# vklyukin/nf_distillation

Measured on NVIDIA B200. Metric: kd_train_samples_per_sec, higher is better.
Workload: dtype bf16

## Files before the change

include/nfk.h:

```cpp
#ifndef NFK_H_
#define NFK_H_

#ifdef __cplusplus
extern "C" {
#endif

#define NFK_OK 0
#define NFK_ERR_SHAPE (-1)
#define NFK_ERR_ALIGN (-2)
#define NFK_ERR_ARG (-3)
#define NFK_ERR_LAUNCH (-4)
#define NFK_ERR_DRIVER (-5)

#define NFK_EPI_F32 0
#define NFK_EPI_BIAS_RELU_BF16 1
#define NFK_EPI_MASK_BF16 2

int nfk_version(void);

int nfk_gemm_nt_bf16(const void* A, long long lda, const void* B, long long ldb, int M, int N, int K, int epi,
                     void* out, long long ldo, const float* bias, const void* aux, long long ldaux, float* colsum,
                     void* stream);

int nfk_gemm_set_prof(void* buf);
// ... 86 lines not shown
                            const float* g_z1_sq, const float* g_ld, float* dx, float* dw, float* dbias, float* dlogs,
                            int B, int C, int H, int W, void* stream);
int nfk_dequant_squeeze(const void* src, int src_is_u8, int n_bits, const float* noise, float* x_out, float* sq_out,
                        int B, int C, int H, int W, void* stream);
int nfk_prior_bpd_fwd(const float* z, const float* mean, const float* logs, const float* logdet, int B, int n,
                      float scale, float* out, void* stream);
int nfk_prior_bpd_bwd(const float* z, const float* mean, const float* logs, const float* g_bpd, int B, int n,
                      float scale, float* dz, float* dlogdet, void* stream);
int nfk_kd_mse_fwd(const float* s, const float* t, int B, int n, float scale, float* acc, void* stream);
int nfk_kd_mse_bwd(const float* s, const float* t, const float* g, int B, int n, float scale, float* ds,
                   int accumulate, void* stream);

int nfk_pconv_coupling_supported(int C, int H, int W, int hid);
int nfk_pconv_coupling_fwd(const void* h2, const void* B3, int K3p, const float* bias3, float* y, float* hsave,
                           float* ld, int B, int C, int H, int W, int hid, int reverse, void* stream);

int nfk_conv1_dgrad_affine_bwd_supported(int C, int H, int W, int hid);
int nfk_conv1_dgrad_affine_bwd(const void* dpre1, const void* B1T, int K1p, const float* dy, const float* x,
                               const float* Wf, float* dx, float* dWf, float* dbf, int B, int C, int H, int W, int hid,
                               void* stream);

int nfk_flow1d_supported(int D, int Cc, int hid, int training);
int nfk_flow1d_sizes(int D, int Cc, int hid, int* total_fwd, int* total_bwd, int* total_grad, int* n_act,
                     int* offsets);
int nfk_flow1d_pack(const float* Wf, const float* bf, const float* const* w, const float* const* b, int D, int Cc,
                    int hid, float* PF, float* PB, void* stream);
int nfk_flow1d_fwd(const float* x, const float* cond, const float* PF, const float* sl, float* y, const float* ld_in,
                   float* ld_out, float* acts, int B, int D, int Cc, int hid, int reverse, void* stream);
int nfk_flow1d_bwd(const float* x_in, const float* cond, const float* acts, const float* PB, const float* y_out,
                   const float* g_out, const float* g_ld, float* dx, float* G, int B, int D, int Cc, int hid,
// ... 80 lines not shown
```

nf_distillation_b200/_lib.py:

```python
from __future__ import annotations

import ctypes
import os

from . import build as _build

_c = ctypes
_vp, _i, _ll, _f = _c.c_void_p, _c.c_int, _c.c_longlong, _c.c_float

ERRORS = {
    -1: "NFK_ERR_SHAPE (unsupported / inconsistent sizes)",
    -2: "NFK_ERR_ALIGN (pointer or leading dimension not 16-byte aligned)",
    -3: "NFK_ERR_ARG (missing / invalid argument)",
    -4: "NFK_ERR_LAUNCH (CUDA launch failure)",
    -5: "NFK_ERR_DRIVER (tensor-map encode failure)",
}



class InvconvItem(_c.Structure):
    _fields_ = [(n, _vp) for n in ("an_bias", "an_logs", "lower", "upper", "log_s", "p", "sign_s", "weight")] + \
               [("C", _i), ("reverse", _i), ("transpose", _i)] + \
               [(n, _vp) for n in ("outW", "outb", "out_sl")]

# ... 54 lines not shown
    "nfk_kd_mse_fwd": [_vp, _vp, _i, _i, _f, _vp, _vp],
    "nfk_kd_mse_bwd": [_vp, _vp, _vp, _i, _i, _f, _vp, _i, _vp],
    "nfk_flow1d_supported": [_i, _i, _i, _i],
    "nfk_flow1d_sizes": [_i, _i, _i, _vp, _vp, _vp, _vp, _vp],
    "nfk_flow1d_pack": [_vp, _vp, _vp, _vp, _i, _i, _i, _vp, _vp, _vp],
    "nfk_flow1d_fwd": [_vp] * 8 + [_i] * 5 + [_vp],
    "nfk_flow1d_bwd": [_vp] * 9 + [_i] * 5 + [_vp],
    "nfk_affine_rows": [_vp] * 7 + [_i, _i, _f, _vp],
    "nfk_gemm_nt_bf16_ranged": [_vp, _ll, _vp, _ll, _i, _i, _i, _i, _vp, _ll, _vp, _vp, _ll, _vp, _i, _vp, _vp, _vp],
    "nfk_cnet_set_prof": [_vp],
    "nfk_cnet_fwd_fused": [_vp, _i, _vp, _vp, _vp, _vp, _vp, _vp, _vp, _vp, _ll, _i, _i, _vp],
    "nfk_cnet_bwd_fused": [_vp, _i, _vp, _vp, _vp, _vp, _ll, _vp, _vp, _vp, _vp, _i, _i, _vp],
    "nfk_cnet_fwd_fused_ranged": [_vp, _i, _vp, _vp, _vp, _vp, _vp, _vp, _vp, _vp, _ll, _i, _i, _i, _vp],
    "nfk_pconv_coupling_supported": [_i, _i, _i, _i],
    "nfk_pconv_coupling_fwd": [_vp, _vp, _i, _vp, _vp, _vp, _vp, _i, _i, _i, _i, _i, _i, _vp],
    "nfk_conv1_dgrad_affine_bwd_supported": [_i, _i, _i, _i],
    "nfk_conv1_dgrad_affine_bwd": [_vp] * 9 + [_i] * 5 + [_vp],
    "nfk_made_prep": [_vp] * 5 + [_i] * 4 + [_vp] * 6 + [_i, _vp],
    "nfk_made_prep_bwd": [_vp] * 5 + [_i] * 3 + [_vp] * 3 + [_vp],
    "nfk_rows_to_bf16": [_vp, _i, _i, _i, _vp, _vp],
    "nfk_made_affine_fwd": [_vp, _vp, _i, _vp, _vp, _i, _vp, _vp, _i, _i, _i, _vp],
    "nfk_made_affine_bwd": [_vp, _vp, _i, _vp, _vp, _vp, _vp, _vp, _i, _i, _i, _vp],
    "nfk_made_inv_update": [_vp, _vp, _i, _vp, _vp, _i, _vp, _vp, _i, _i, _i, _i, _i, _vp],
    "nfk_made_inverse_resident_supported": [_i, _i, _i],
    "nfk_made_inverse_push_supported": [_i, _i, _i, _i],
    "nfk_made_inverse_jobs": [_vp, _vp, _i, _i, _i, _i, _i, _vp, _i],
    "nfk_made_inverse_pack": [_vp, _i, _vp, _vp, _vp, _i, _i, _i, _i, _i, _vp, _vp],
    "nfk_made_inverse_resident": [_vp] * 6 + [_i] * 3 + [_vp] * 3 + [_i] * 6 + [_vp],
    "nfk_kd_nll_loss_scratch_floats": [_i],
    "nfk_kd_nll_loss_fwd": [_vp, _vp, _i, _vp, _vp, _vp, _f, _vp, _vp, _vp, _f, _f, _f, _i, _vp, _vp, _vp, _vp, _vp],
# ... 49 lines not shown
```

nf_distillation_b200/csrc/pconv_coupling.cu:

```cuda
#include <cuda.h>
#include <cuda_bf16.h>
#include <cuda_runtime.h>
#include <cstdint>
#include <cstdlib>

#include "../../include/nfk.h"
#include "launch_util.h"
#include "ptx.cuh"

namespace nfk {

constexpr int PC_EPI = 384;
constexpr int PC_THREADS = 64 + PC_EPI;
constexpr int PC_BK = 64;

template <int C> struct PcCfg;
template <> struct PcCfg<12> { static constexpr int NPIX = 256, MB = 1, WIN = 160, STAGES = 3; };
template <> struct PcCfg<24> { static constexpr int NPIX = 128, MB = 2, WIN = 64, STAGES = 3; };
template <> struct PcCfg<48> { static constexpr int NPIX = 64, MB = 4, WIN = 32, STAGES = 2; };

struct PcArgs {
  long long M;
  int num_kb;
  int B, H, W, lgHW, lgW;
  const float* bias3;
  float* y;
  float* hsave;
  float* ld;
  int reverse;
  int banded, nb, rb;
};

template <int NPIX>
__device__ __forceinline__ long long pc_tile_pix0(const PcArgs& g, int t) {
  if (!g.banded) return static_cast<long long>(t) * NPIX;
  const int img = t / g.nb, band = t - img * g.nb;
  return (static_cast<long long>(img) << g.lgHW) + static_cast<long long>(band * g.rb - 1) * g.W;
}

template <int C>
struct PcSmem {
  using Cfg = PcCfg<C>;
  static constexpr int a_bytes = Cfg::MB * 128 * 128;
  static constexpr int b_bytes = Cfg::NPIX * 128;
  static constexpr int stage_bytes = a_bytes + b_bytes;
  static constexpr int pitch = Cfg::WIN + 1;
  static constexpr int s_bytes = ((9 * C * pitch * 4 + 15) / 16) * 16;
  static constexpr int off_s = Cfg::STAGES * stage_bytes;
  static constexpr int off_bar = off_s + s_bytes;
  static constexpr int off_bias = off_bar + 128;
  static constexpr int total = off_bias + 128;
};

template <int C>
__global__ void __launch_bounds__(PC_THREADS, 1)
pconv_coupling_kernel(const __grid_constant__ CUtensorMap tmW, const __grid_constant__ CUtensorMap tmH,
                      const PcArgs g) {
  using Cfg = PcCfg<C>;
  using Sm = PcSmem<C>;
  constexpr int NPIX = Cfg::NPIX, MB = Cfg::MB, WIN = Cfg::WIN, HALF = NPIX / 2, PC_STAGES = Cfg::STAGES;
  constexpr int K3 = 9 * C, J = C / 2;
  constexpr int ACC_COLS = MB * NPIX;
  extern __shared__ __align__(1024) uint8_t smem[];
  pdl_launch_dependents();
  if (smem_u32(smem) & 1023u) __trap();
  const int warp = static_cast<int>(uniform_u32(threadIdx.x >> 5)), lane = threadIdx.x & 31;
  float* S = reinterpret_cast<float*>(smem + Sm::off_s);
  uint64_t* full = reinterpret_cast<uint64_t*>(smem + Sm::off_bar);
  uint64_t* empty = full + PC_STAGES;
// ... 1 lines not shown
  uint64_t* tmem_empty = tmem_full + 2;
  uint32_t* tmem_slot = reinterpret_cast<uint32_t*>(tmem_empty + 2);
  float* bias_s = reinterpret_cast<float*>(smem + Sm::off_bias);

  const int num_tiles = g.banded ? g.B * g.nb : static_cast<int>((g.M + NPIX - 1) / NPIX);
  if (warp == 0 && lane == 0) {
    tma_prefetch_desc(&tmW);
    tma_prefetch_desc(&tmH);
    for (int s = 0; s < PC_STAGES; ++s) { mbar_init(&full[s], 1); mbar_init(&empty[s], 1); }
    for (int a = 0; a < 2; ++a) { mbar_init(&tmem_full[a], 1); mbar_init(&tmem_empty[a], 8); }
    fence_mbar_init();
  }
  if (warp == 1) { tmem_alloc(tmem_slot, 512); tmem_relinquish(); }
  pdl_wait();
  if (threadIdx.x < C) bias_s[threadIdx.x] = g.bias3[threadIdx.x];
  tc_fence_before();
  __syncthreads();
  tc_fence_after();
  const uint32_t tmem_base = uniform_u32(*tmem_slot);

  if (warp == 0) {
    {
      int s = 0;
      uint32_t ph = 0;
      for (int t = blockIdx.x; t < num_tiles; t += gridDim.x) {
        for (int kb = 0; kb < g.num_kb; ++kb) {
          mbar_wait_warp(&empty[s], ph ^ 1);
          uint8_t* sa = smem + s * Sm::stage_bytes;
          mbar_expect_tx_elect(&full[s], Sm::stage_bytes);
#pragma unroll
// ... 30 lines not shown
          umma_commit_elect(&empty[s]);
          if (++s == PC_STAGES) { s = 0; ph ^= 1; }
        }
        umma_commit_elect(&tmem_full[acc]);
      }
    }
  } else {
    const int q = warp & 3, half = (warp - 2) >> 2;
    const int et = threadIdx.x - 64;
    const bool drains = half < 2;
    const bool banded = (C == 12) && g.banded;
    const int HW = g.H * g.W, HWm = HW - 1, Wm = g.W - 1;
    constexpr int ITEMS = J * NPIX / PC_EPI;
    static_assert(J * NPIX % (2 * PC_EPI) == 0, "each half's items must divide over the epilogue threads");
    const int OH = banded ? (g.rb >> 1) * g.W : HALF;
    int it = 0;
    for (int t = blockIdx.x; t < num_tiles; t += gridDim.x, ++it) {
      const int acc = it & 1;
      const long long tile_base = pc_tile_pix0<NPIX>(g, t);
      const int row0 = banded ? (t % g.nb) * g.rb - 1 : 0;
      const int row_end = banded ? min(g.H, row0 + 1 + g.rb) : 0;
      auto decode = [&](int hf, int ih, int& j, int& pl, long long& m) -> bool {
        j = ih / OH;
        pl = (banded ? g.W : 0) + hf * OH + (ih - j * OH);
        m = tile_base + pl;
        if (j >= J) return false;
        if (!banded) return m < g.M;
        return row0 + (pl >> g.lgW) < row_end;
      };
      float z2v[ITEMS];
#pragma unroll
      for (int k = 0; k < ITEMS; ++k) {
        const int hf = k / (ITEMS / 2);
        int j, pl;
        long long m;
        const bool live = decode(hf, et + PC_EPI * (k - hf * (ITEMS / 2)), j, pl, m);
        const int b = static_cast<int>(m >> g.lgHW), rem = static_cast<int>(m) & HWm;
        z2v[k] = live ? g.y[((static_cast<long long>(b) * C + J + j) << g.lgHW) + rem] : 0.f;
      }
      mbar_wait(&tmem_full[acc], (it >> 1) & 1);
      tc_fence_after();
#pragma unroll
      for (int hf = 0; hf < 2; ++hf) {
        const int w0 = (WIN == HALF) ? hf * HALF : (hf == 0 ? 0 : NPIX - WIN);
        if (hf == 1) asm volatile("bar.sync 1, %0;" ::"n"(PC_EPI) : "memory");
        constexpr int HCOLS = WIN / 2;
        static_assert(HCOLS % 16 == 0, "window halves are drained 16 columns at a time");
#pragma unroll
        for (int mb = 0; mb < MB; ++mb) {
          const int row = mb * 128 + q * 32 + lane;
          const uint32_t taddr = tmem_base + (static_cast<uint32_t>(q * 32) << 16) + acc * ACC_COLS + mb * NPIX + w0 +
                                 half * HCOLS;
          float* srow = S + row * Sm::pitch + half * HCOLS;
// ... 40 lines not shown
              const int dy = tap / 3 - 1, dx = tap % 3 - 1;
              const int ny = yy + dy, nx = xx + dx;
              if (ny >= 0 && ny < g.H && nx >= 0 && nx < g.W) {
                const float* p = sp + tap * C * Sm::pitch + dy * g.W + dx;
                sh += p[0];
                lg += p[Sm::pitch];
              }
            }
            if (g.hsave) *reinterpret_cast<float2*>(g.hsave + m * C + 2 * j) = make_float2(sh, lg);
            const float tt = lg + 2.f;
            const float e = expf(-fabsf(tt));
            const float l1p = log1pf(e);
            float sg, lsv;
            if (tt >= 0.f) { sg = 1.f / (1.f + e); lsv = -l1p; }
            else { sg = e / (1.f + e); lsv = tt - l1p; }
            g.y[((static_cast<long long>(b) * C + J + j) << g.lgHW) + rem] =
                g.reverse ? (z2v[k] / sg - sh) : (z2v[k] + sh) * sg;
            lsum = g.reverse ? -lsv : lsv;
          }
          if (g.ld) {
            const int seg = HW < 32 ? HW : 32;
#pragma unroll
            for (int o = 16; o > 0; o >>= 1) {
              const float v = __shfl_xor_sync(0xffffffffu, lsum, o);
              if (o < seg) lsum += v;
            }
            if ((lane & (seg - 1)) == 0 && live) atomicAdd(g.ld + b, lsum);
          }
        }
      }
      asm volatile("bar.sync 1, %0;" ::"n"(PC_EPI) : "memory");
    }
  }
  tc_fence_before();
  __syncthreads();
  if (warp == 1) tmem_dealloc(tmem_base, 512);
}

typedef CUresult (*EncodeTiledFn3)(CUtensorMap*, CUtensorMapDataType, cuuint32_t, void*, const cuuint64_t*,
                                   const cuuint64_t*, const cuuint32_t*, const cuuint32_t*, CUtensorMapInterleave,
                                   CUtensorMapSwizzle, CUtensorMapL2promotion, CUtensorMapFloatOOBfill);

int pc_tmap(CUtensorMap* m, const void* ptr, uint64_t cols, uint64_t rows, uint64_t ld, uint32_t box_rows) {
// ... 5 lines not shown
        q != cudaDriverEntryPointSuccess)
      return NFK_ERR_DRIVER;
    fn = reinterpret_cast<EncodeTiledFn3>(p);
  }
  if ((reinterpret_cast<uintptr_t>(ptr) & 15) || (ld * 2) % 16) return NFK_ERR_ALIGN;
  cuuint64_t dims[2] = {cols, rows};
  cuuint64_t strides[1] = {ld * 2};
  cuuint32_t box[2] = {64, box_rows};
  cuuint32_t estr[2] = {1, 1};
  CUresult r = fn(m, CU_TENSOR_MAP_DATA_TYPE_BFLOAT16, 2, const_cast<void*>(ptr), dims, strides, box, estr,
                  CU_TENSOR_MAP_INTERLEAVE_NONE, CU_TENSOR_MAP_SWIZZLE_128B, CU_TENSOR_MAP_L2_PROMOTION_L2_256B,
                  CU_TENSOR_MAP_FLOAT_OOB_FILL_NONE);
  return r == CUDA_SUCCESS ? NFK_OK : NFK_ERR_DRIVER;
}

template <int C>
static int pc_launch(const void* h2, const void* B3, int K3p, const PcArgs& g, int hid, cudaStream_t st) {
  using Cfg = PcCfg<C>;
  CUtensorMap tmW, tmH;
  int rc;
  if ((rc = pc_tmap(&tmW, B3, hid, K3p, hid, 128))) return rc;
  if ((rc = pc_tmap(&tmH, h2, hid, static_cast<uint64_t>(g.M), hid, Cfg::NPIX))) return rc;
  if ((rc = ensure_dyn_smem(reinterpret_cast<const void*>(pconv_coupling_kernel<C>), PcSmem<C>::total))) return rc;
  int dev = 0, sms = 148;
  cudaGetDevice(&dev);
  cudaDeviceGetAttribute(&sms, cudaDevAttrMultiProcessorCount, dev);
  const int tiles = g.banded ? g.B * g.nb : static_cast<int>((g.M + Cfg::NPIX - 1) / Cfg::NPIX);
  const cudaError_t le = launch_pdl(pconv_coupling_kernel<C>, dim3(tiles < sms ? tiles : sms), dim3(PC_THREADS),
                                    PcSmem<C>::total, st, tmW, tmH, g);
  return (le == cudaSuccess && cudaGetLastError() == cudaSuccess) ? NFK_OK : NFK_ERR_LAUNCH;
}

int pconv_px_launch(const void* h2, const void* B3, int K3p, const float* bias3, float* y, float* hsave, float* ld,
                    int B, int C, int hid, int reverse, cudaStream_t st);
static bool pconv_use_px() {
  static const bool v = [] { const char* e = getenv("NFK_PCONV_PX"); return !(e && e[0] == '0'); }();
  return v;
}

}

using namespace nfk;

extern "C" int nfk_pconv_coupling_supported(int C, int H, int W, int hid) {
  if (hid <= 0 || hid % 64) return 0;
  const int HW = H * W;
  if (HW < 4 || (HW & (HW - 1)) || (W & (W - 1))) return 0;
  if (C == 12) {
    if (HW <= PcCfg<12>::NPIX / 2) return 1;
    if (HW == PcCfg<12>::NPIX && W + 1 <= PcCfg<12>::WIN - PcCfg<12>::NPIX / 2) return 1;
    return W * 8 == PcCfg<12>::NPIX && 3 * W + W + 1 <= PcCfg<12>::WIN + 1;
  }
  if (C == 24) return HW <= PcCfg<24>::NPIX / 2 && HW >= 4;
  if (C == 48) return HW <= PcCfg<48>::NPIX / 2 && HW >= 4;
  if (C == 96) return H == 4 && W == 4 && pconv_use_px();
  return 0;
}

extern "C" int nfk_pconv_coupling_fwd(const void* h2, const void* B3, int K3p, const float* bias3, float* y,
                                      float* hsave, float* ld, int B, int C, int H, int W, int hid, int reverse,
                                      void* stream) {
  if (B <= 0 || !nfk_pconv_coupling_supported(C, H, W, hid)) return NFK_ERR_SHAPE;
  if (K3p % 64 || K3p < 9 * C || K3p > 128 * ((9 * C + 127) / 128)) return NFK_ERR_SHAPE;
  if (!h2 || !B3 || !bias3 || !y) return NFK_ERR_ARG;
  PcArgs g{};
  g.M = static_cast<long long>(B) * H * W;
  g.num_kb = hid / 64;
  g.B = B; g.H = H; g.W = W;
  g.lgW = 0; while ((1 << g.lgW) < W) ++g.lgW;
  g.lgHW = 0; while ((1 << g.lgHW) < H * W) ++g.lgHW;
  g.bias3 = bias3; g.y = y; g.hsave = hsave; g.ld = ld; g.reverse = reverse;
// ... 13 lines not shown
```

nf_distillation_b200/functional.py:

```python
from __future__ import annotations

import os
from dataclasses import dataclass
from typing import Optional

import torch

from . import ops

BF16 = torch.bfloat16
F32 = torch.float32
USE_FUSED_CNET = os.environ.get("NFK_FUSED_CNET", "1") != "0"
USE_FUSED_PCONV = os.environ.get("NFK_FUSED_PCONV", "1") != "0"
USE_FUSED_CNET_BWD = os.environ.get("NFK_FUSED_CNET_BWD", "1") != "0"
USE_FUSED_DGRAD1 = os.environ.get("NFK_FUSED_DGRAD1", "1") != "0"

WGRAD_STREAM_MAX_M = int(os.environ.get("NFK_WGRAD_STREAM_MAX_M", "65536"))
_wgrad_streams: dict = {}
_wgrad_keepalive: list = []


def _wgrad_stream(dev):
    key = (dev.type, dev.index if dev.index is not None else torch.cuda.current_device())
    st = _wgrad_streams.get(key)
    if st is None:
        st = _wgrad_streams[key] = torch.cuda.Stream(device=dev)
    return st


def _join_wgrads(dev):
# ... 41 lines not shown


class PrepCtx:

    def __init__(self, steps, reverse: bool):
        self.steps = list(steps)
        self.reverse = bool(reverse)
        self.index = {id(s): i for i, s in enumerate(self.steps)}
        n = len(self.steps)
        self.consts = [None] * n
        self.items = [None] * n
        self.grads = [None] * n
        self.cops = [None] * n
        self.citems = [None] * n
        self.cgrads = [None] * n
        self.token = None

    def build(self):
        flat = []
        for st in self.steps:
            iv = st.invconv
            if iv.LU_decomposed:
                flat += [st.actnorm.bias, st.actnorm.logs, iv.lower, iv.upper, iv.log_s]
            else:
                flat += [st.actnorm.bias, st.actnorm.logs, iv.weight, iv.weight, iv.weight]
        for st in self.steps:
            if not st.is_1d:
                flat += list(st._coupling_params_2d())
        self.token = PrepAllFn.apply(self, *flat)
        return self
# ... 174 lines not shown
        ops.gemm_nt(col, k.B1, M, hid, K1p, ops.EPI_BIAS_RELU_BF16, h1, bias=k.bias1, aux=m1)
        ops.gemm_nt(h1, k.B2, M, hid, hid, ops.EPI_BIAS_RELU_BF16, h2, bias=k.bias2, aux=m2)
    return (h1, h2, m1, m2) if keep else (None, h2, None, None)


def _conv3_coupling(h2, k: StepConsts, y, hsave, ld, B, C, H, W, hid, K3p, reverse):
    M = B * H * W
    if USE_FUSED_PCONV and ops.pconv_coupling_supported(C, H, W, hid):
        ops.pconv_coupling_fwd(h2, k.B3, K3p, k.bias3, y, hsave, ld, B, C, H, W, hid, reverse)
        return
    P = torch.empty(M, K3p, device=h2.device, dtype=F32)
    ops.gemm_nt(h2, k.B3, M, K3p, hid, ops.EPI_F32, P)
    ops.coupling_fwd(P, K3p, k.bias3, y, hsave, ld, B, C, H, W, reverse=reverse)


def flowstep2d_forward(x, ld_in, k: StepConsts, hid, keep):
    B, C, H, W = x.shape
    M, cin = B * H * W, C // 2
    K1p, K3p = ops.round_up(9 * cin, 64), ops.round_up(9 * C, 64)
    dev = x.device
    y = torch.empty_like(x)
    col = torch.empty(M, K1p, device=dev, dtype=BF16)
    ld_out = torch.empty(B, device=dev, dtype=F32)
    ops.affine1x1_fwd(x, k.Wf, k.bf, k.sl, y, col, K1p, ld_in, ld_out, B, C, H, W)
    h1, h2, m1, m2 = _coupling_net(col, k, M, hid, K1p, K3p, keep)
    hsave = torch.empty(M, C, device=dev, dtype=F32) if keep else None
    _conv3_coupling(h2, k, y, hsave, ld_out, B, C, H, W, hid, K3p, False)
    return y, ld_out, (col, h1, h2 if keep else None, hsave, m1, m2)


def flowstep2d_reverse(z, ld_in, k: StepConsts, hid, keep=False):
    B, C, H, W = z.shape
    M, cin = B * H * W, C // 2
    K1p, K3p = ops.round_up(9 * cin, 64), ops.round_up(9 * C, 64)
    dev = z.device
    col = torch.empty(M, K1p, device=dev, dtype=BF16)
    ops.affine1x1_fwd(z, None, None, None, None, col, K1p, None, None, B, C, H, W)
    h1, h2, m1, m2 = _coupling_net(col, k, M, hid, K1p, K3p, keep)
    hsave = torch.empty(M, C, device=dev, dtype=F32) if keep else None
    zc = z.clone()
    ld_mid = ld_in.clone()
    _conv3_coupling(h2, k, zc, hsave, ld_mid, B, C, H, W, hid, K3p, True)
# ... 38 lines not shown
        ops.gemm_tn(dhcol, h2, K3p, hid, M, dB3)
        ops.gemm_tn(dpre2, h1, hid, hid, M, dB2)
        ops.gemm_tn(dpre1, col, hid, K1p, M, dB1)
    return dpre1


def _conv1_dgrad(dpre1, B1T, M, K1p, hid):
    dcol = torch.empty(M, K1p, device=dpre1.device, dtype=F32)
    ops.gemm_nt(dpre1, B1T, M, K1p, hid, ops.EPI_F32, dcol)
    return dcol


class FlowStep2dFn(torch.autograd.Function):

    @staticmethod
    def forward(ctx, x, ld_in, hid, token, pctx, idx):
        B, C, H, W = x.shape
        x = x.contiguous()
        Wf, bf, sl = pctx.consts[idx]
        k = StepConsts(Wf, bf, sl, *pctx.cops[idx])
        y, ld_out, (col, h1, h2, hsave, m1, m2) = flowstep2d_forward(x, ld_in.contiguous(), k, hid, keep=True)
        ctx.hid = hid
        ctx.pctx, ctx.idx = pctx, idx
        ctx.save_for_backward(x, y, col, h1, h2, hsave, m1, m2, Wf, k.B1T, k.B2T, k.B3T)
        return y, ld_out

    @staticmethod
    def backward(ctx, g_out, g_ld):
        (x, z_out, col, h1, h2, hsave, m1, m2, Wf, B1T, B2T, B3T) = ctx.saved_tensors
        hid = ctx.hid
        B, C, H, W = x.shape
        M, cin = B * H * W, C // 2
        K1p, K3p = ops.round_up(9 * cin, 64), ops.round_up(9 * C, 64)
        dev = x.device
        _join_wgrads(dev)
        g_out = torch.zeros_like(x) if g_out is None else g_out.contiguous()
# ... 2 lines not shown

        dy = torch.empty_like(x)
        dhcol = torch.empty(M, K3p, device=dev, dtype=BF16)
        ops.coupling_bwd(g_out, g_ld, z_out, hsave, dy, dhcol, K3p, dbias3, B, C, H, W)
        dpre1 = _coupling_net_backward(dhcol, col, h1, h2, m1, m2, B1T, B2T, B3T, dbias2, dbias1, dB3, dB2, dB1, arena,
                                       M, hid, K1p, K3p)
        dx = torch.empty_like(x)
        if USE_FUSED_DGRAD1 and ops.conv1_dgrad_affine_bwd_supported(C, H, W, hid):
            ops.conv1_dgrad_affine_bwd(dpre1, B1T, K1p, dy, x, Wf, dx, dWf, dbf, B, C, H, W, hid)
        else:
            dcol = _conv1_dgrad(dpre1, B1T, M, K1p, hid)
            ops.affine1x1_bwd(dy, dcol, K1p, x, Wf, dx, dWf, dbf, B, C, H, W)

        ctx.pctx.grads[ctx.idx] = (dWf, C, dbf, g_ld, B, float(H * W))
        ctx.pctx.cgrads[ctx.idx] = (dB1, dbias1, dB2, dbias2, dB3, dbias3)
        return (dx, g_ld, None, None, None, None)


class FlowStep2dReverseFn(torch.autograd.Function):

    @staticmethod
    def forward(ctx, z, ld_in, hid, token, pctx, idx):
        z = z.contiguous()
        Wf, bf, sl = pctx.consts[idx]
        k = StepConsts(Wf, bf, sl, *pctx.cops[idx])
        x, ld_out, (zc, col, h1, h2, hsave, m1, m2) = flowstep2d_reverse(z, ld_in.contiguous(), k, hid, keep=True)
        ctx.hid = hid
        ctx.pctx, ctx.idx = pctx, idx
        ctx.save_for_backward(zc, col, h1, h2, hsave, m1, m2, Wf, k.B1T, k.B2T, k.B3T)
        return x, ld_out

# ... 206 lines not shown
```

nf_distillation_b200/models/flows.py:

```python
from __future__ import annotations

import logging
import math

import torch
import torch.nn as nn

from .. import functional as Fn
from .layers import (ActNorm1d, ActNorm2d, Conv2d, Conv2dZeros, InvertibleConv1x1, LinearZeros, Permute2d, Split2d,
                     SqueezeLayer, _as_logdet, _require_cuda, gaussian_likelihood, gaussian_sample)
from .utils import (can_fuse_dequant_squeeze, dequantize_and_squeeze, split_feature,
                    uniform_binning_correction)

logger = logging.getLogger(__name__)


def get_block_2d(in_channels, out_channels, hidden_channels):
    return nn.Sequential(
        Conv2d(in_channels, hidden_channels),
        nn.ReLU(inplace=False),
        Conv2d(hidden_channels, hidden_channels, kernel_size=(1, 1)),
        nn.ReLU(inplace=False),
        Conv2dZeros(hidden_channels, out_channels),
    )
# ... 147 lines not shown
                    f"256) run on the tensor-core GEMM path instead; training them is not built.")
        if not self.is_1d:
            if self.condition_features:
                raise NotImplementedError("y-conditioned 2-D coupling is not built (no shipped image config uses it)")
            if self.hidden_channels % 64 or self.in_channels not in (12, 24, 48, 96):
                raise NotImplementedError("2-D FlowStep kernels need hidden_channels % 64 == 0 and "
                                          "C in {12, 24, 48, 96}")
            if not self.invconv.LU_decomposed and torch.is_grad_enabled():
                pass

    def forward(self, input, y_onehot=None, logdet=None, reverse=False):
        self._check_supported(input)
        if self.is_1d:
            from .. import flow1d
            return flow1d.flowstep1d(self, input, y_onehot, logdet, reverse)
        B = input.shape[0]
        ld = _as_logdet(logdet, B, input.device)
        want_ld = ld is not None
        if ld is None:
            ld = torch.zeros(B, device=input.device)
        params = self._all_params()
        needs_grad = torch.is_grad_enabled() and (input.requires_grad or ld.requires_grad
                                                  or any(p.requires_grad for p in params))
        if self.precision == "bf16x3":
            return self._forward_precise(input, ld, want_ld, reverse, needs_grad)
        if not reverse:
            if needs_grad:
                pctx, idx, token = Fn.prep_for(self, False)
                z, ld_out = Fn.FlowStep2dFn.apply(input, ld, self.hidden_channels, token, pctx, idx)
            else:
                z, ld_out, _ = Fn.flowstep2d_forward(input.contiguous(), ld.contiguous(), self._consts(False),
                                                     self.hidden_channels, keep=False)
        else:
            if needs_grad:
                pctx, idx, token = Fn.prep_for(self, True)
                z, ld_out = Fn.FlowStep2dReverseFn.apply(input, ld, self.hidden_channels, token, pctx, idx)
            else:
                z, ld_out = Fn.flowstep2d_reverse(input.contiguous(), ld.contiguous(), self._consts(True),
                                                  self.hidden_channels)
        return z, (ld_out if want_ld else None)

    def _forward_precise(self, input, ld, want_ld, reverse, needs_grad):
        from .. import precise
        if self.flow_coupling != "affine":
            raise NotImplementedError("bf16x3 precision is built for the affine coupling")
        with torch.set_grad_enabled(needs_grad):
            fp = precise.folded_params(self)
            if not reverse:
                z, ld_out = precise.FlowStep2dX3Fn.apply(input, ld, self.hidden_channels, *fp)
            else:
                if needs_grad:
                    raise NotImplementedError("gradients through the 2-D inverse pass are built for the bf16 "
                                              "precision only")
                k = self._consts(True)
                z, ld_out = precise.flowstep2d_reverse_x3(input.contiguous(), ld.contiguous(), self.hidden_channels,
# ... 33 lines not shown
                                            condition_features=condition_features))
                self.output_shapes.append([-1, C] if is_1d else [-1, C, H, W])
            if i < L - 1 and not is_1d:
                self.layers.append(Split2d(num_channels=C))
                self.output_shapes.append([-1, C // 2, H, W])
                C = C // 2

    def forward(self, input, y_onehot=None, logdet=0.0, reverse=False, temperature=None, _sq0=None):
        if reverse:
            return self.decode(input, y_onehot=y_onehot, temperature=temperature)
        return self.encode(input, y_onehot=y_onehot, logdet=logdet, _sq0=_sq0)

    def _encode_layers(self, z, y_onehot, logdet, sq0=None):
        layers = self.layers
        i, n = 0, len(layers)
        while i < n:
            layer = layers[i]
            if i == 0 and sq0 is not None and isinstance(layer, SqueezeLayer) and layer.factor == 2:
                z = sq0
                yield z, logdet
                i += 1
                continue
            nxt = layers[i + 1] if i + 1 < n else None
            if (isinstance(layer, Split2d) and isinstance(nxt, SqueezeLayer) and nxt.factor == 2
                    and z.shape[2] % 2 == 0 and z.shape[3] % 2 == 0):
                z1, z, logdet = layer.forward_with_squeeze(z, logdet=logdet)
                yield z1, logdet
                yield z, logdet
                i += 2
                continue
            z, logdet = layer(z, y_onehot=y_onehot, logdet=logdet, reverse=False)
            yield z, logdet
            i += 1

    def encode(self, z, y_onehot=None, logdet=0.0, _sq0=None):
        with Fn.use_prep(Fn.prepare_steps(self.layers, False)):
            for z, logdet in self._encode_layers(z, y_onehot, logdet, _sq0):
                pass
        return z, logdet

    def decode(self, z, y_onehot=None, temperature=None):
        with Fn.use_prep(Fn.prepare_steps(self.layers, True)):
            for layer in reversed(self.layers):
                if isinstance(layer, Split2d):
                    z, _ = layer(z, logdet=0, reverse=True, temperature=temperature)
                else:
# ... 108 lines not shown
```

nf_distillation_b200/ops.py:

```python
from __future__ import annotations

import ctypes

import torch

from ._lib import LIB, check

EPI_F32, EPI_BIAS_RELU_BF16, EPI_MASK_BF16 = 0, 1, 2

_LAUNCHES = 0


def launch_count() -> int:
    return _LAUNCHES


def _p(t):
    if t is None:
        return None
    assert t.is_cuda and t.is_contiguous(), "libnfk needs contiguous CUDA tensors"
    return t.data_ptr()


def _st():
# ... 216 lines not shown

def kd_mse_bwd(s, t, g, B, n, scale, ds, accumulate=False):
    _count()
    check(LIB.nfk_kd_mse_bwd(_p(s), _p(t), _p(g), B, n, float(scale), _p(ds), int(accumulate), _st()),
          "nfk_kd_mse_bwd")


def pconv_coupling_supported(C, H, W, hid):
    return bool(LIB.nfk_pconv_coupling_supported(C, H, W, hid))


def pconv_coupling_fwd(h2, B3, K3p, bias3, y, hsave, ld, B, C, H, W, hid, reverse):
    _count()
    check(LIB.nfk_pconv_coupling_fwd(_p(h2), _p(B3), K3p, _p(bias3), _p(y), _p(hsave), _p(ld), B, C, H, W, hid,
                                     int(reverse), _st()), "nfk_pconv_coupling_fwd")


def conv1_dgrad_affine_bwd_supported(C, H, W, hid):
    return bool(LIB.nfk_conv1_dgrad_affine_bwd_supported(C, H, W, hid))


def conv1_dgrad_affine_bwd(dpre1, B1T, K1p, dy, x, Wf, dx, dWf, dbf, B, C, H, W, hid):
    assert dpre1.dtype == torch.bfloat16 and B1T.dtype == torch.bfloat16
    _count()
    check(LIB.nfk_conv1_dgrad_affine_bwd(_p(dpre1), _p(B1T), K1p, _p(dy), _p(x), _p(Wf), _p(dx), _p(dWf), _p(dbf), B,
                                         C, H, W, hid, _st()), "nfk_conv1_dgrad_affine_bwd")


def flow1d_supported(D, Cc, hid, training=False):
    return bool(LIB.nfk_flow1d_supported(D, Cc, hid, int(training)))
# ... 189 lines not shown
```

Baseline: 55030.

## Fuse next flow step's affine 1x1 and im2col into coupling conv3 epilogue

```diff
diff --git a/include/nfk.h b/include/nfk.h
--- a/include/nfk.h
+++ b/include/nfk.h
@@ -124,6 +124,11 @@
 int nfk_pconv_coupling_supported(int C, int H, int W, int hid);
 int nfk_pconv_coupling_fwd(const void* h2, const void* B3, int K3p, const float* bias3, float* y, float* hsave,
                            float* ld, int B, int C, int H, int W, int hid, int reverse, void* stream);
+int nfk_pconv_coupling_chain_supported(int C, int H, int W, int hid);
+int nfk_pconv_coupling_fwd_chain(const void* h2, const void* B3, int K3p, const float* bias3, float* y, float* hsave,
+                                 float* ld, int B, int C, int H, int W, int hid, const float* Wn, const float* bn,
+                                 const float* sln, float* y_next, void* col_next, int K1p, float* ld_next,
+                                 void* stream);
 
 int nfk_conv1_dgrad_affine_bwd_supported(int C, int H, int W, int hid);
 int nfk_conv1_dgrad_affine_bwd(const void* dpre1, const void* B1T, int K1p, const float* dy, const float* x,
diff --git a/nf_distillation_b200/_lib.py b/nf_distillation_b200/_lib.py
--- a/nf_distillation_b200/_lib.py
+++ b/nf_distillation_b200/_lib.py
@@ -92,6 +92,9 @@
     "nfk_cnet_fwd_fused_ranged": [_vp, _i, _vp, _vp, _vp, _vp, _vp, _vp, _vp, _vp, _ll, _i, _i, _i, _vp],
     "nfk_pconv_coupling_supported": [_i, _i, _i, _i],
     "nfk_pconv_coupling_fwd": [_vp, _vp, _i, _vp, _vp, _vp, _vp, _i, _i, _i, _i, _i, _i, _vp],
+    "nfk_pconv_coupling_chain_supported": [_i, _i, _i, _i],
+    "nfk_pconv_coupling_fwd_chain": [_vp, _vp, _i, _vp, _vp, _vp, _vp, _i, _i, _i, _i, _i, _vp, _vp, _vp, _vp, _vp,
+                                     _i, _vp, _vp],
     "nfk_conv1_dgrad_affine_bwd_supported": [_i, _i, _i, _i],
     "nfk_conv1_dgrad_affine_bwd": [_vp] * 9 + [_i] * 5 + [_vp],
     "nfk_made_prep": [_vp] * 5 + [_i] * 4 + [_vp] * 6 + [_i, _vp],
diff --git a/nf_distillation_b200/csrc/pconv_coupling.cu b/nf_distillation_b200/csrc/pconv_coupling.cu
--- a/nf_distillation_b200/csrc/pconv_coupling.cu
+++ b/nf_distillation_b200/csrc/pconv_coupling.cu
@@ -29,6 +29,12 @@
   float* ld;
   int reverse;
   int banded, nb, rb;
+  const float* Wn;
+  const float* bn;
+  const float* sln;
+  float* y_next;
+  __nv_bfloat16* col_next;
+  float* ld_next;
 };
 
 template <int NPIX>
@@ -50,9 +56,16 @@
   static constexpr int off_bar = off_s + s_bytes;
   static constexpr int off_bias = off_bar + 128;
   static constexpr int total = off_bias + 128;
+  static constexpr int off_wn = total;
+  static constexpr int total_chain = off_wn + (((C * C + C) * 4 + 15) / 16) * 16;
 };
 
-template <int C>
+__device__ __forceinline__ uint32_t pc_bf2(float lo, float hi) {
+  __nv_bfloat162 v = __floats2bfloat162_rn(lo, hi);
+  return *reinterpret_cast<uint32_t*>(&v);
+}
+
+template <int C, bool CHAIN>
 __global__ void __launch_bounds__(PC_THREADS, 1)
 pconv_coupling_kernel(const __grid_constant__ CUtensorMap tmW, const __grid_constant__ CUtensorMap tmH,
                       const PcArgs g) {
@@ -84,6 +97,11 @@
   if (warp == 1) { tmem_alloc(tmem_slot, 512); tmem_relinquish(); }
   pdl_wait();
   if (threadIdx.x < C) bias_s[threadIdx.x] = g.bias3[threadIdx.x];
+  float* wn_s = reinterpret_cast<float*>(smem + Sm::off_wn);
+  if constexpr (CHAIN) {
+    for (int i = threadIdx.x; i < C * C; i += PC_THREADS) wn_s[i] = g.Wn[i];
+    if (threadIdx.x < C) wn_s[C * C + threadIdx.x] = g.bn[threadIdx.x];
+  }
   tc_fence_before();
   __syncthreads();
   tc_fence_after();
@@ -144,6 +162,20 @@
     constexpr int ITEMS = J * NPIX / PC_EPI;
     static_assert(J * NPIX % (2 * PC_EPI) == 0, "each half's items must divide over the epilogue threads");
     const int OH = banded ? (g.rb >> 1) * g.W : HALF;
+    constexpr int CW = C == 12 ? 16 : 8, K1 = 9 * J, K1P = (K1 + 63) / 64 * 64, R16 = K1P / 8, ZP = NPIX + 1;
+    static_assert(PC_EPI % R16 == 0, "a thread packs one chunk column");
+    int eoff[8], erow[8], ecol[8];
+    if constexpr (CHAIN) {
+      const int c4 = et & (R16 - 1);
+#pragma unroll
+      for (int e = 0; e < 8; ++e) {
+        const int k = c4 * 8 + e, tap = k / J, ci = k - tap * J;
+        const bool real = k < K1;
+        erow[e] = real ? tap / 3 : 3;
+        ecol[e] = real ? tap % 3 : 3;
+        eoff[e] = real ? ci * ZP + (tap / 3 - 1) * CW + (tap % 3 - 1) : 0;
+      }
+    }
     int it = 0;
     for (int t = blockIdx.x; t < num_tiles; t += gridDim.x, ++it) {
       const int acc = it & 1;
@@ -159,6 +191,7 @@
         return row0 + (pl >> g.lgW) < row_end;
       };
       float z2v[ITEMS];
+      float z1v[CHAIN ? ITEMS : 1];
 #pragma unroll
       for (int k = 0; k < ITEMS; ++k) {
         const int hf = k / (ITEMS / 2);
@@ -167,6 +200,7 @@
         const bool live = decode(hf, et + PC_EPI * (k - hf * (ITEMS / 2)), j, pl, m);
         const int b = static_cast<int>(m >> g.lgHW), rem = static_cast<int>(m) & HWm;
         z2v[k] = live ? g.y[((static_cast<long long>(b) * C + J + j) << g.lgHW) + rem] : 0.f;
+        if constexpr (CHAIN) z1v[k] = live ? g.y[((static_cast<long long>(b) * C + j) << g.lgHW) + rem] : 0.f;
       }
       mbar_wait(&tmem_full[acc], (it >> 1) & 1);
       tc_fence_after();
@@ -237,8 +271,9 @@
             float sg, lsv;
             if (tt >= 0.f) { sg = 1.f / (1.f + e); lsv = -l1p; }
             else { sg = e / (1.f + e); lsv = tt - l1p; }
-            g.y[((static_cast<long long>(b) * C + J + j) << g.lgHW) + rem] =
-                g.reverse ? (z2v[k] / sg - sh) : (z2v[k] + sh) * sg;
+            const float zn = g.reverse ? (z2v[k] / sg - sh) : (z2v[k] + sh) * sg;
+            g.y[((static_cast<long long>(b) * C + J + j) << g.lgHW) + rem] = zn;
+            if constexpr (CHAIN) z2v[k] = zn;
             lsum = g.reverse ? -lsv : lsv;
           }
           if (g.ld) {
@@ -250,6 +285,71 @@
             }
             if ((lane & (seg - 1)) == 0 && live) atomicAdd(g.ld + b, lsum);
           }
+        }
+      }
+      if constexpr (CHAIN) {
+        static_assert(C != 12 || NPIX == 256, "chained C = 12: one 16x16 image per tile");
+        static_assert(C * ZP + J * ZP <= 9 * C * Sm::pitch, "z tile and y_next[:, :C/2] fit the staging window");
+        float* Zs = S;
+        float* Y1s = S + C * ZP;
+        asm volatile("bar.sync 1, %0;" ::"n"(PC_EPI) : "memory");
+#pragma unroll
+        for (int k = 0; k < ITEMS; ++k) {
+          const int hf = k / (ITEMS / 2);
+          int j, pl;
+          long long m;
+          if (decode(hf, et + PC_EPI * (k - hf * (ITEMS / 2)), j, pl, m)) {
+            Zs[j * ZP + pl] = z1v[k];
+            Zs[(J + j) * ZP + pl] = z2v[k];
+          }
+        }
+        if (et < (NPIX >> g.lgHW)) {
+          const long long b = (tile_base >> g.lgHW) + et;
+          if (b < g.B) g.ld_next[b] = __ldcg(g.ld + b) + g.sln[0] * static_cast<float>(HW);
+        }
+        asm volatile("bar.sync 1, %0;" ::"n"(PC_EPI) : "memory");
+        constexpr int OPG = C / 3;
+#pragma unroll 1
+        for (int i = et; i < 3 * NPIX; i += PC_EPI) {
+          const int pl = i & (NPIX - 1), grp = i / NPIX;
+          const long long m = tile_base + pl;
+          if (m >= g.M) continue;
+          float zr[C];
+#pragma unroll
+          for (int c = 0; c < C; ++c) zr[c] = Zs[c * ZP + pl];
+          const int b = static_cast<int>(m >> g.lgHW), rem = static_cast<int>(m) & HWm;
+          float* yp = g.y_next + ((static_cast<long long>(b) * C) << g.lgHW) + rem;
+#pragma unroll
+          for (int oo = 0; oo < OPG; ++oo) {
+            const int o = grp * OPG + oo;
+            float acc = wn_s[C * C + o];
+            const float4* wr = reinterpret_cast<const float4*>(wn_s + o * C);
+#pragma unroll
+            for (int c = 0; c < C / 4; ++c) {
+              const float4 w = wr[c];
+              acc = fmaf(w.x, zr[4 * c], acc);
+              acc = fmaf(w.y, zr[4 * c + 1], acc);
+              acc = fmaf(w.z, zr[4 * c + 2], acc);
+              acc = fmaf(w.w, zr[4 * c + 3], acc);
+            }
+            yp[static_cast<long long>(o) << g.lgHW] = acc;
+            if (o < J) Y1s[o * ZP + pl] = acc;
+          }
+        }
+        asm volatile("bar.sync 1, %0;" ::"n"(PC_EPI) : "memory");
+        uint4* col4 = reinterpret_cast<uint4*>(g.col_next) + tile_base * R16;
+#pragma unroll 1
+        for (int i = et; i < NPIX * R16; i += PC_EPI) {
+          const int pl = i / R16;
+          if (tile_base + pl >= g.M) continue;
+          const int yy = (pl / CW) % CW, xx = pl % CW;
+          const uint32_t rm = (yy > 0 ? 1u : 0u) | 2u | (yy < CW - 1 ? 4u : 0u);
+          const uint32_t cm = (xx > 0 ? 1u : 0u) | 2u | (xx < CW - 1 ? 4u : 0u);
+          const float* yb = Y1s + pl;
+          float v[8];
+#pragma unroll
+          for (int e = 0; e < 8; ++e) v[e] = ((rm >> erow[e]) & (cm >> ecol[e]) & 1u) ? yb[eoff[e]] : 0.f;
+          col4[i] = make_uint4(pc_bf2(v[0], v[1]), pc_bf2(v[2], v[3]), pc_bf2(v[4], v[5]), pc_bf2(v[6], v[7]));
         }
       }
       asm volatile("bar.sync 1, %0;" ::"n"(PC_EPI) : "memory");
@@ -285,20 +385,21 @@
   return r == CUDA_SUCCESS ? NFK_OK : NFK_ERR_DRIVER;
 }
 
-template <int C>
+template <int C, bool CHAIN = false>
 static int pc_launch(const void* h2, const void* B3, int K3p, const PcArgs& g, int hid, cudaStream_t st) {
   using Cfg = PcCfg<C>;
   CUtensorMap tmW, tmH;
   int rc;
   if ((rc = pc_tmap(&tmW, B3, hid, K3p, hid, 128))) return rc;
   if ((rc = pc_tmap(&tmH, h2, hid, static_cast<uint64_t>(g.M), hid, Cfg::NPIX))) return rc;
-  if ((rc = ensure_dyn_smem(reinterpret_cast<const void*>(pconv_coupling_kernel<C>), PcSmem<C>::total))) return rc;
+  constexpr int smem = CHAIN ? PcSmem<C>::total_chain : PcSmem<C>::total;
+  if ((rc = ensure_dyn_smem(reinterpret_cast<const void*>(pconv_coupling_kernel<C, CHAIN>), smem))) return rc;
   int dev = 0, sms = 148;
   cudaGetDevice(&dev);
   cudaDeviceGetAttribute(&sms, cudaDevAttrMultiProcessorCount, dev);
   const int tiles = g.banded ? g.B * g.nb : static_cast<int>((g.M + Cfg::NPIX - 1) / Cfg::NPIX);
-  const cudaError_t le = launch_pdl(pconv_coupling_kernel<C>, dim3(tiles < sms ? tiles : sms), dim3(PC_THREADS),
-                                    PcSmem<C>::total, st, tmW, tmH, g);
+  const cudaError_t le = launch_pdl(pconv_coupling_kernel<C, CHAIN>, dim3(tiles < sms ? tiles : sms), dim3(PC_THREADS),
+                                    smem, st, tmW, tmH, g);
   return (le == cudaSuccess && cudaGetLastError() == cudaSuccess) ? NFK_OK : NFK_ERR_LAUNCH;
 }
 
@@ -326,6 +427,34 @@
   if (C == 48) return HW <= PcCfg<48>::NPIX / 2 && HW >= 4;
   if (C == 96) return H == 4 && W == 4 && pconv_use_px();
   return 0;
+}
+
+extern "C" int nfk_pconv_coupling_chain_supported(int C, int H, int W, int hid) {
+  if (!nfk_pconv_coupling_supported(C, H, W, hid)) return 0;
+  return (C == 12 && H == 16 && W == 16) || (C == 24 && H == 8 && W == 8);
+}
+
+extern "C" int nfk_pconv_coupling_fwd_chain(const void* h2, const void* B3, int K3p, const float* bias3, float* y,
+                                            float* hsave, float* ld, int B, int C, int H, int W, int hid,
+                                            const float* Wn, const float* bn, const float* sln, float* y_next,
+                                            void* col_next, int K1p, float* ld_next, void* stream) {
+  if (B <= 0 || !nfk_pconv_coupling_chain_supported(C, H, W, hid)) return NFK_ERR_SHAPE;
+  if (K3p % 64 || K3p < 9 * C || K3p > 128 * ((9 * C + 127) / 128)) return NFK_ERR_SHAPE;
+  if (K1p != (9 * (C / 2) + 63) / 64 * 64) return NFK_ERR_SHAPE;
+  if (!h2 || !B3 || !bias3 || !y || !ld || !Wn || !bn || !sln || !y_next || !col_next || !ld_next) return NFK_ERR_ARG;
+  if ((reinterpret_cast<uintptr_t>(Wn) | reinterpret_cast<uintptr_t>(col_next)) & 15) return NFK_ERR_ALIGN;
+  PcArgs g{};
+  g.M = static_cast<long long>(B) * H * W;
+  g.num_kb = hid / 64;
+  g.B = B; g.H = H; g.W = W;
+  g.lgW = 0; while ((1 << g.lgW) < W) ++g.lgW;
+  g.lgHW = 0; while ((1 << g.lgHW) < H * W) ++g.lgHW;
+  g.bias3 = bias3; g.y = y; g.hsave = hsave; g.ld = ld;
+  g.Wn = Wn; g.bn = bn; g.sln = sln; g.y_next = y_next; g.col_next = static_cast<__nv_bfloat16*>(col_next);
+  g.ld_next = ld_next;
+  cudaStream_t st = static_cast<cudaStream_t>(stream);
+  if (C == 12) return pc_launch<12, true>(h2, B3, K3p, g, hid, st);
+  return pc_launch<24, true>(h2, B3, K3p, g, hid, st);
 }
 
 extern "C" int nfk_pconv_coupling_fwd(const void* h2, const void* B3, int K3p, const float* bias3, float* y,
diff --git a/nf_distillation_b200/functional.py b/nf_distillation_b200/functional.py
--- a/nf_distillation_b200/functional.py
+++ b/nf_distillation_b200/functional.py
@@ -14,6 +14,8 @@
 USE_FUSED_PCONV = os.environ.get("NFK_FUSED_PCONV", "1") != "0"
 USE_FUSED_CNET_BWD = os.environ.get("NFK_FUSED_CNET_BWD", "1") != "0"
 USE_FUSED_DGRAD1 = os.environ.get("NFK_FUSED_DGRAD1", "1") != "0"
+USE_CHAIN_AFFINE = os.environ.get("NFK_CHAIN_AFFINE", "1") != "0"
+CHAIN_MAX_M = 16384
 
 WGRAD_STREAM_MAX_M = int(os.environ.get("NFK_WGRAD_STREAM_MAX_M", "65536"))
 _wgrad_streams: dict = {}
@@ -85,6 +87,7 @@
         self.cops = [None] * n
         self.citems = [None] * n
         self.cgrads = [None] * n
+        self.chain = None
         self.token = None
 
     def build(self):
@@ -289,18 +292,36 @@
     ops.coupling_fwd(P, K3p, k.bias3, y, hsave, ld, B, C, H, W, reverse=reverse)
 
 
-def flowstep2d_forward(x, ld_in, k: StepConsts, hid, keep):
+def chains(B, C, H, W, hid):
+    return (USE_CHAIN_AFFINE and USE_FUSED_PCONV and B * H * W <= CHAIN_MAX_M
+            and ops.pconv_coupling_chain_supported(C, H, W, hid))
+
+
+def step_buffers(x):
+    B, C, H, W = x.shape
+    K1p = ops.round_up(9 * (C // 2), 64)
+    return (torch.empty_like(x), torch.empty(B * H * W, K1p, device=x.device, dtype=BF16),
+            torch.empty(B, device=x.device, dtype=F32))
+
+
+def flowstep2d_forward(x, ld_in, k: StepConsts, hid, keep, pre=None, nxt=None):
     B, C, H, W = x.shape
     M, cin = B * H * W, C // 2
     K1p, K3p = ops.round_up(9 * cin, 64), ops.round_up(9 * C, 64)
     dev = x.device
-    y = torch.empty_like(x)
-    col = torch.empty(M, K1p, device=dev, dtype=BF16)
-    ld_out = torch.empty(B, device=dev, dtype=F32)
-    ops.affine1x1_fwd(x, k.Wf, k.bf, k.sl, y, col, K1p, ld_in, ld_out, B, C, H, W)
+    if pre is None:
+        y, col, ld_out = step_buffers(x)
+        ops.affine1x1_fwd(x, k.Wf, k.bf, k.sl, y, col, K1p, ld_in, ld_out, B, C, H, W)
+    else:
+        y, col, ld_out = pre
     h1, h2, m1, m2 = _coupling_net(col, k, M, hid, K1p, K3p, keep)
     hsave = torch.empty(M, C, device=dev, dtype=F32) if keep else None
-    _conv3_coupling(h2, k, y, hsave, ld_out, B, C, H, W, hid, K3p, False)
+    if nxt is None:
+        _conv3_coupling(h2, k, y, hsave, ld_out, B, C, H, W, hid, K3p, False)
+    else:
+        kn, y_n, col_n, ld_n = nxt
+        ops.pconv_coupling_fwd_chain(h2, k.B3, K3p, k.bias3, y, hsave, ld_out, B, C, H, W, hid, kn.Wf, kn.bf, kn.sl,
+                                     y_n, col_n, K1p, ld_n)
     return y, ld_out, (col, h1, h2 if keep else None, hsave, m1, m2)
 
 
@@ -369,12 +390,25 @@
 class FlowStep2dFn(torch.autograd.Function):
 
     @staticmethod
-    def forward(ctx, x, ld_in, hid, token, pctx, idx):
+    def forward(ctx, x, ld_in, hid, token, pctx, idx, nidx=None):
         B, C, H, W = x.shape
         x = x.contiguous()
+        ld_in = ld_in.contiguous()
         Wf, bf, sl = pctx.consts[idx]
         k = StepConsts(Wf, bf, sl, *pctx.cops[idx])
-        y, ld_out, (col, h1, h2, hsave, m1, m2) = flowstep2d_forward(x, ld_in.contiguous(), k, hid, keep=True)
+        pre, pctx.chain = pctx.chain, None
+        if pre is not None:
+            p_idx, p_y, p_ld, p_ver, bufs = pre
+            ok = (p_idx == idx and x.data_ptr() == p_y.data_ptr() and x._version == p_ver
+                  and ld_in.data_ptr() == p_ld.data_ptr())
+            pre = bufs if ok else None
+        nxt = None
+        if nidx is not None and chains(B, C, H, W, hid):
+            Wn, bn, sln = pctx.consts[nidx]
+            nxt = (StepConsts(Wn, bn, sln), *step_buffers(x))
+        y, ld_out, (col, h1, h2, hsave, m1, m2) = flowstep2d_forward(x, ld_in, k, hid, keep=True, pre=pre, nxt=nxt)
+        if nxt is not None:
+            pctx.chain = (nidx, y, ld_out, y._version, nxt[1:])
         ctx.hid = hid
         ctx.pctx, ctx.idx = pctx, idx
         ctx.save_for_backward(x, y, col, h1, h2, hsave, m1, m2, Wf, k.B1T, k.B2T, k.B3T)
@@ -407,7 +441,7 @@
 
         ctx.pctx.grads[ctx.idx] = (dWf, C, dbf, g_ld, B, float(H * W))
         ctx.pctx.cgrads[ctx.idx] = (dB1, dbias1, dB2, dbias2, dB3, dbias3)
-        return (dx, g_ld, None, None, None, None)
+        return (dx, g_ld, None, None, None, None, None)
 
 
 class FlowStep2dReverseFn(torch.autograd.Function):
diff --git a/nf_distillation_b200/models/flows.py b/nf_distillation_b200/models/flows.py
--- a/nf_distillation_b200/models/flows.py
+++ b/nf_distillation_b200/models/flows.py
@@ -185,6 +185,20 @@
         if self.is_1d:
             from .. import flow1d
             return flow1d.flowstep1d(self, input, y_onehot, logdet, reverse)
+        z, ld_out, _ = self._forward_2d(input, logdet, reverse)
+        return z, ld_out
+
+    def _chains_to(self, nxt) -> bool:
+        return (isinstance(nxt, FlowStep) and not self.is_1d and not nxt.is_1d and not nxt.condition_features
+                and self.precision == "bf16" and nxt.precision == "bf16" and nxt.in_channels == self.in_channels
+                and nxt.hidden_channels == self.hidden_channels and nxt.actnorm.inited
+                and nxt.block[0].actnorm.inited and nxt.block[2].actnorm.inited)
+
+    def forward_chained(self, input, logdet, pre, nxt):
+        self._check_supported(input)
+        return self._forward_2d(input, logdet, False, pre, nxt)
+
+    def _forward_2d(self, input, logdet, reverse, pre=None, nxt=None):
         B = input.shape[0]
         ld = _as_logdet(logdet, B, input.device)
         want_ld = ld is not None
@@ -194,14 +208,22 @@
         needs_grad = torch.is_grad_enabled() and (input.requires_grad or ld.requires_grad
                                                   or any(p.requires_grad for p in params))
         if self.precision == "bf16x3":
-            return self._forward_precise(input, ld, want_ld, reverse, needs_grad)
+            return (*self._forward_precise(input, ld, want_ld, reverse, needs_grad), None)
+        pre_next = None
         if not reverse:
             if needs_grad:
                 pctx, idx, token = Fn.prep_for(self, False)
-                z, ld_out = Fn.FlowStep2dFn.apply(input, ld, self.hidden_channels, token, pctx, idx)
+                nidx = pctx.lookup(nxt, False) if nxt is not None else None
+                z, ld_out = Fn.FlowStep2dFn.apply(input, ld, self.hidden_channels, token, pctx, idx, nidx)
             else:
-                z, ld_out, _ = Fn.flowstep2d_forward(input.contiguous(), ld.contiguous(), self._consts(False),
-                                                     self.hidden_channels, keep=False)
+                x = input.contiguous()
+                chain = None
+                if (nxt is not None and Fn.chains(*x.shape, self.hidden_channels)
+                        and not (torch.is_grad_enabled() and any(p.requires_grad for p in nxt._all_params()))):
+                    pre_next = Fn.step_buffers(x)
+                    chain = (nxt._consts(False), *pre_next)
+                z, ld_out, _ = Fn.flowstep2d_forward(x, ld.contiguous(), self._consts(False), self.hidden_channels,
+                                                     keep=False, pre=pre, nxt=chain)
         else:
             if needs_grad:
                 pctx, idx, token = Fn.prep_for(self, True)
@@ -209,7 +231,7 @@
             else:
                 z, ld_out = Fn.flowstep2d_reverse(input.contiguous(), ld.contiguous(), self._consts(True),
                                                   self.hidden_channels)
-        return z, (ld_out if want_ld else None)
+        return z, (ld_out if want_ld else None), pre_next
 
     def _forward_precise(self, input, ld, want_ld, reverse, needs_grad):
         from .. import precise
@@ -273,6 +295,7 @@
     def _encode_layers(self, z, y_onehot, logdet, sq0=None):
         layers = self.layers
         i, n = 0, len(layers)
+        pre = None
         while i < n:
             layer = layers[i]
             if i == 0 and sq0 is not None and isinstance(layer, SqueezeLayer) and layer.factor == 2:
@@ -288,7 +311,10 @@
                 yield z, logdet
                 i += 2
                 continue
-            z, logdet = layer(z, y_onehot=y_onehot, logdet=logdet, reverse=False)
+            if isinstance(layer, FlowStep) and not layer.is_1d:
+                z, logdet, pre = layer.forward_chained(z, logdet, pre, nxt if layer._chains_to(nxt) else None)
+            else:
+                z, logdet = layer(z, y_onehot=y_onehot, logdet=logdet, reverse=False)
             yield z, logdet
             i += 1
 
diff --git a/nf_distillation_b200/ops.py b/nf_distillation_b200/ops.py
--- a/nf_distillation_b200/ops.py
+++ b/nf_distillation_b200/ops.py
@@ -254,6 +254,18 @@
     _count()
     check(LIB.nfk_pconv_coupling_fwd(_p(h2), _p(B3), K3p, _p(bias3), _p(y), _p(hsave), _p(ld), B, C, H, W, hid,
                                      int(reverse), _st()), "nfk_pconv_coupling_fwd")
+
+
+def pconv_coupling_chain_supported(C, H, W, hid):
+    return bool(LIB.nfk_pconv_coupling_chain_supported(C, H, W, hid))
+
+
+def pconv_coupling_fwd_chain(h2, B3, K3p, bias3, y, hsave, ld, B, C, H, W, hid, Wn, bn, sln, y_next, col_next, K1p,
+                             ld_next):
+    _count()
+    check(LIB.nfk_pconv_coupling_fwd_chain(_p(h2), _p(B3), K3p, _p(bias3), _p(y), _p(hsave), _p(ld), B, C, H, W, hid,
+                                           _p(Wn), _p(bn), _p(sln), _p(y_next), _p(col_next), K1p, _p(ld_next),
+                                           _st()), "nfk_pconv_coupling_fwd_chain")
 
 
 def conv1_dgrad_affine_bwd_supported(C, H, W, hid):
```

Result: no change. 55230 (median of 6 runs) (+0.4%).
